# cloudflare/zkp-ecdsa

Measured on NVIDIA H100. Metric: ZKAttest proofs/sec, higher is better.
Workload: dtype u256/u258 (32-bit limbs, Montgomery)

## Files before the change

__graft_entry__.py:

```python
from __future__ import annotations

import hashlib
import os
import subprocess
import sys

ROOT = os.path.dirname(os.path.abspath(__file__))
CSRC = os.path.join(ROOT, 'zkp_ecdsa_b200', 'csrc')
LIB = os.path.join(ROOT, 'zkp_ecdsa_b200', 'libzkattest.so')
LIB_WAR = os.path.join(ROOT, 'zkp_ecdsa_b200', 'libzkattest_war256.so')
HOSTSIM = os.path.join(ROOT, 'tests', 'hostsim', 'libzkattest_hostsim.so')
HOSTSIM_WAR = os.path.join(ROOT, 'tests', 'hostsim', 'libzkattest_hostsim_war256.so')
PROBE_SRC = os.path.join(ROOT, 'tests', 'probe', 'zk_probe.cu')
PROBE = os.path.join(ROOT, 'tests', 'probe', 'libzkprobe.so')
PROBE_HOST = os.path.join(ROOT, 'tests', 'probe', 'libzkprobe_host.so')
ORACLE_CPU = os.path.join(ROOT, 'oracle', '_ref', 'libzkattest_cpu.so')
ARCH = ['-gencode', 'arch=compute_90a,code=sm_90a']
NVCC_FLAGS = ARCH + ['-O3', '-std=c++17', '-lineinfo',
              '--compiler-options', '-fPIC', '-shared']


def _sources():
    return sorted(os.path.join(CSRC, f) for f in os.listdir(CSRC) if f.endswith(('.cu', '.cuh', '.h', '.inc')))


def _stamp(extra='', files=()):
    h = hashlib.sha256(extra.encode())
    for p in _sources() + [os.path.join(ROOT, 'include', 'zkattest.h')] + list(files):
        h.update(p.encode())
        h.update(open(p, 'rb').read())
    return h.hexdigest()


def _build_if_stale(out, cmd, tag, files=()):
    stamp_file = out + '.stamp'
    stamp = _stamp(' '.join(cmd), files)
    if os.path.exists(out) and os.path.exists(stamp_file) and open(stamp_file).read() == stamp:
        return False
    print(f'[build] {tag}: {" ".join(cmd)}', flush=True)
    tmp = out + '.tmp'
    subprocess.check_call([tmp if c == out else c for c in cmd], cwd=ROOT)
    os.replace(tmp, out)
    open(stamp_file, 'w').write(stamp)
    return True


def build_lib():
    nvcc = os.environ.get('NVCC', '/usr/local/cuda/bin/nvcc')
    cmd = [nvcc] + NVCC_FLAGS + ['-I' + os.path.join(ROOT, 'include'), '-I' + CSRC, '-o', LIB,
                                 os.path.join(CSRC, 'zkattest.cu')]
    return _build_if_stale(LIB, cmd, 'libzkattest.so (sm_90a)')


def build_lib_war():
    nvcc = os.environ.get('NVCC', '/usr/local/cuda/bin/nvcc')
    cmd = [nvcc] + NVCC_FLAGS + ['-DZKA_PG_WAR256', '-I' + os.path.join(ROOT, 'include'), '-I' + CSRC, '-o', LIB_WAR,
                                 os.path.join(CSRC, 'zkattest.cu')]
    return _build_if_stale(LIB_WAR, cmd, 'libzkattest_war256.so (sm_90a)')


def build_hostsim(war=False):
    out = HOSTSIM_WAR if war else HOSTSIM
    os.makedirs(os.path.dirname(out), exist_ok=True)
    cmd = ['g++', '-std=c++17', '-O2', '-DZKA_HOSTSIM'] + (['-DZKA_PG_WAR256'] if war else []) + [
        '-x', 'c++', '-I' + os.path.join(ROOT, 'include'), '-I' + CSRC, '-fPIC', '-shared', '-o', out,
        os.path.join(CSRC, 'zkattest.cu')]
    return _build_if_stale(out, cmd, 'hostsim war256 (tests only)' if war else 'hostsim (tests only)')


def build_probe(host=False):
    out = PROBE_HOST if host else PROBE
    if host:
        cmd = ['g++', '-std=c++17', '-O2', '-DZKA_HOSTSIM', '-x', 'c++', '-fPIC', '-shared']
    else:
        cmd = [os.environ.get('NVCC', '/usr/local/cuda/bin/nvcc')] + NVCC_FLAGS
    cmd += ['-I' + os.path.join(ROOT, 'include'), '-I' + CSRC, '-o', out, PROBE_SRC]
    return _build_if_stale(out, cmd, 'probe host (tests only)' if host else 'probe (sm_90a, tests only)', [PROBE_SRC])


def build_oracle_cpu():
    src = os.path.join(ROOT, 'oracle', 'cpu', 'zkattest_cpu.cpp')
    hdr = os.path.join(ROOT, 'include', 'zkattest.h')
    if os.path.exists(ORACLE_CPU) and os.path.getmtime(ORACLE_CPU) >= max(os.path.getmtime(src), os.path.getmtime(hdr)):
        return False
    print('[build] oracle/cpu -> oracle/_ref/libzkattest_cpu.so', flush=True)
    subprocess.check_call(['make', '-C', os.path.join(ROOT, 'oracle', 'cpu')])
    return True


def build_tools():
    nvcc = os.environ.get('NVCC', '/usr/local/cuda/bin/nvcc')
    tdir = os.path.join(ROOT, 'tools')
    for name in ('imad_peak', 'mul_peak'):
        src, out = os.path.join(tdir, name + '.cu'), os.path.join(tdir, name)
        if not os.path.exists(src):
            continue
        if os.path.exists(out) and os.path.getmtime(out) >= max(os.path.getmtime(p) for p in _sources() + [src]):
            continue
        cmd = [nvcc] + ARCH + ['-O3', '-std=c++17', '-I' + CSRC,
               '-I' + os.path.join(ROOT, 'include'), '-o', out, src]
        print(f'[build] tools/{name}: {" ".join(cmd)}', flush=True)
        subprocess.check_call(cmd, cwd=ROOT)


def build() -> None:
    from concurrent.futures import ThreadPoolExecutor
    jobs = [build_lib, build_lib_war, build_hostsim, lambda: build_hostsim(war=True), build_oracle_cpu, build_tools,
            build_probe, lambda: build_probe(host=True)]
    with ThreadPoolExecutor(max_workers=min(len(jobs), max(1, (os.cpu_count() or 2)))) as ex:
        for f in [ex.submit(j) for j in jobs]:
            f.result()
    sys.path.insert(0, ROOT)
    import zkp_ecdsa_b200
    import oracle


def smoke() -> None:
    sys.path.insert(0, ROOT)
    import numpy as np
    from zkp_ecdsa_b200 import api, synth
    from oracle import flat
    from oracle import zkattest as OZ
    from oracle.big import Tape

    eng = api.Engine(device=0)
    rnd = synth.params_rnd(1)
    params = eng.generate_params_list(rnd=rnd)
    wl = synth.Workload(B=2, N=8, seed=1)
    tape = synth.random_tape(2, eng.lib.prove_tape_len(8), seed=2)
    res = eng.prove_batch(params, wl.msg_hash, wl.sig, wl.pk, wl.which, wl.ring, tape)
    assert (res.status == 0).all(), res.status
    oparams = OZ.generate_params_list(Tape(rnd))
    for b in range(2):
        pr = OZ.prove_signature_list(oparams, wl.msg_hash[b].tobytes(), wl.sig[b].tobytes(), wl.pk[b].tobytes(),
                                     int(wl.which[b]), wl.ring_ints(), Tape(tape[b].tobytes()))
        assert flat.ser_proof(pr) == res.proof_bytes(b), f'proof {b} differs from the oracle'
    from zkp_ecdsa_b200 import verify_tape as VT
    vts = eng.lib.verify_tape_len(8, 80)
    ok = np.zeros(2, np.uint8)
    st = np.zeros(2, np.int32)
    eng.lib.verify_batch(params.handle, 2, wl.msg_hash, wl.ring, 8, res.proofs, res.proofs.shape[1], res.proof_len,
                         VT.random_verify_tape(2, vts, 8, 80, seed=3), vts, ok, st)
    assert list(ok) == [1, 1] and not st.any(), (ok, st)
    launched = eng.lib.launch_count()
    war = ''
    if os.path.exists(LIB_WAR):
        from oracle.curves import tomEdwards256, war256
        ew = api.Engine(device=0, proof_group='war256')
        pw = ew.generate_params_list(16, rnd=rnd)
        tw = synth.random_tape(1, ew.lib.prove_tape_len(8, 16), seed=4)
        rw = ew.prove_batch(pw, wl.msg_hash[:1], wl.sig[:1], wl.pk[:1], wl.which[:1], wl.ring, tw)
        assert (rw.status == 0).all(), rw.status
        flat.set_proof_group(war256)
        try:
            ow = OZ.generate_params_list(Tape(rnd), 16, war256)
            pr = OZ.prove_signature_list(ow, wl.msg_hash[0].tobytes(), wl.sig[0].tobytes(), wl.pk[0].tobytes(),
                                         int(wl.which[0]), wl.ring_ints(), Tape(tw[0].tobytes()))
            assert flat.ser_proof(pr) == rw.proof_bytes(0), 'war256 proof differs from the oracle'
        finally:
            flat.set_proof_group(tomEdwards256)
        launched += ew.lib.launch_count()
        war = '; war256 build: 1 proof bit-exact'
    print(f'smoke ok: 2 proofs bit-exact vs oracle and accepted by the verifier{war}; kernels launched:', launched)


if __name__ == '__main__':
    build()
    if len(sys.argv) > 1 and sys.argv[1] == 'smoke':
        smoke()
```

zkp_ecdsa_b200/csrc/zk_field.cuh:

```cuda
#pragma once
#include <stdint.h>
#include "zk_field_consts.inc"

#if defined(__CUDACC__)
#define ZK_HD __host__ __device__ __forceinline__
#define ZK_HDN __host__ __device__ __noinline__
#else
#define ZK_HD inline __attribute__((always_inline))
#define ZK_HDN __attribute__((noinline))
#endif

namespace zk {

#define ZK_FIELD_DESC(NAME, PFX, NL, LAZY)                                   \
  struct NAME {                                                              \
    static constexpr int N = NL;                                             \
    static constexpr bool kLazy = LAZY;                                      \
    static constexpr uint32_t kN0Inv = PFX##_N0INV;                          \
    ZK_HD static constexpr uint32_t p(int i) {                               \
      constexpr uint32_t t[NL] = PFX##_P;                                    \
      return t[i];                                                           \
    }                                                                        \
    ZK_HD static constexpr uint32_t rr(int i) {                              \
      constexpr uint32_t t[NL] = PFX##_RR;                                   \
// ... 135 lines not shown
      uint32_t c = add_n<N>(s, a, b);
      uint32_t br = sub_p<F>(t, s);
      csel_n<N>(r, (c != 0) || (br == 0), t, s);
    }
  }
  ZK_HD static void sub(uint32_t* r, const uint32_t* a, const uint32_t* b) {
    if (F::kLazy) {
      uint32_t p8[N];
#pragma unroll
      for (int i = 0; i < N; i++) p8[i] = (F::p(i) << 3) | (i > 0 ? (F::p(i - 1) >> 29) : 0u);
      uint32_t t[N];
      add_n<N>(t, a, p8);
      sub_n<N>(r, t, b);
    } else {
      uint32_t s[N], t[N];
      uint32_t br = sub_n<N>(s, a, b);
      uint32_t pp[N];
#pragma unroll
      for (int i = 0; i < N; i++) pp[i] = F::p(i);
      add_n<N>(t, s, pp);
      csel_n<N>(r, br != 0, t, s);
    }
  }
  ZK_HD static void neg(uint32_t* r, const uint32_t* a) {
    uint32_t z[N];
    zero_n<N>(z);
    sub(r, z, a);
  }
  ZK_HD static void dbl(uint32_t* r, const uint32_t* a) { add(r, a, a); }

  ZK_HD static void mul(uint32_t* r, const uint32_t* a, const uint32_t* b) {
#if defined(__CUDA_ARCH__) && !defined(ZKA_NO_PTX_MUL)
    if (same_t<F, FpTom>::value) { ptx::tom_mul(r, a, b); return; }
    if (same_t<F, FpP256>::value) { ptx::p256_mul(r, a, b); return; }
    if (same_t<F, FpWar>::value) {
      ptx::V8 x, y;
#pragma unroll
      for (int i = 0; i < 8; i++) { x.v[i] = a[i]; y.v[i] = b[i]; }
      const ptx::V8 z = ptx::cios8_mul_fn<FpWar>(x, y);
#pragma unroll
      for (int i = 0; i < 8; i++) r[i] = z.v[i];
      return;
    }
#endif
    mul_generic(r, a, b);
  }
  ZK_HD static void mul_generic(uint32_t* r, const uint32_t* a, const uint32_t* b) {
    uint32_t t[N + 2];
#pragma unroll
    for (int i = 0; i < N + 2; i++) t[i] = 0;
#pragma unroll
    for (int i = 0; i < N; i++) {
      uint64_t c = 0;
      const uint32_t bi = b[i];
#pragma unroll
      for (int j = 0; j < N; j++) {
        uint64_t s = (uint64_t)a[j] * bi + t[j] + c;
        t[j] = (uint32_t)s;
        c = s >> 32;
      }
      uint64_t s = (uint64_t)t[N] + c;
      t[N] = (uint32_t)s;
      t[N + 1] = (uint32_t)(s >> 32);
      const uint32_t m = t[0] * F::kN0Inv;
      c = ((uint64_t)m * F::p(0) + t[0]) >> 32;
#pragma unroll
      for (int j = 1; j < N; j++) {
        uint64_t s2 = (uint64_t)m * F::p(j) + t[j] + c;
        t[j - 1] = (uint32_t)s2;
        c = s2 >> 32;
      }
      s = (uint64_t)t[N] + c;
      t[N - 1] = (uint32_t)s;
      t[N] = t[N + 1] + (uint32_t)(s >> 32);
    }
    if (F::kLazy) {
      copy_n<N>(r, t);
    } else {
      uint32_t u[N];
      uint32_t br = sub_p<F>(u, t);
      csel_n<N>(r, (t[N] != 0) || (br == 0), u, t);
    }
  }
  ZK_HD static void sqr(uint32_t* r, const uint32_t* a) { mul(r, a, a); }

  ZK_HD static void set_one(uint32_t* r) {
#pragma unroll
    for (int i = 0; i < N; i++) r[i] = F::one(i);
  }
  ZK_HD static void to_mont(uint32_t* r, const uint32_t* a) {
    uint32_t rr[N];
#pragma unroll
    for (int i = 0; i < N; i++) rr[i] = F::rr(i);
    mul(r, a, rr);
  }
  ZK_HD static void from_mont(uint32_t* r, const uint32_t* a) {
    uint32_t o[N];
    zero_n<N>(o);
    o[0] = 1;
    mul(r, a, o);
    if (F::kLazy) {
      uint32_t t[N], p2[N];
#pragma unroll
      for (int i = 0; i < N; i++) p2[i] = (F::p(i) << 1) | (i > 0 ? (F::p(i - 1) >> 31) : 0u);
      uint32_t br = sub_n<N>(t, r, p2);
      csel_n<N>(r, br == 0, t, r);
      br = sub_p<F>(t, r);
      csel_n<N>(r, br == 0, t, r);
    } else {
      reduce(r);
    }
  }
  ZK_HD static bool is_zero(const uint32_t* a) {
    uint32_t t[N];
    copy_n<N>(t, a);
    reduce(t);
    return is_zero_n<N>(t);
  }
  ZK_HD static bool eq(const uint32_t* a, const uint32_t* b) {
    uint32_t t[N], u[N];
    copy_n<N>(t, a);
    copy_n<N>(u, b);
    reduce(t);
    reduce(u);
    return eq_n<N>(t, u);
  }

  static ZK_HDN void inv_fermat(uint32_t* r, const uint32_t* a) {
    uint32_t e[N];
#pragma unroll
    for (int i = 0; i < N; i++) e[i] = F::p(i);
    e[0] -= 2;
    uint32_t acc[N], base[N];
    set_one(acc);
    copy_n<N>(base, a);
    int top = N * 32 - 1;
    while (top > 0 && !((e[top >> 5] >> (top & 31)) & 1)) top--;
#pragma unroll 1
    for (int bit = top; bit >= 0; bit--) {
      sqr(acc, acc);
      if ((e[bit >> 5] >> (bit & 31)) & 1) mul(acc, acc, base);
    }
    copy_n<N>(r, acc);
  }

  static ZK_HDN void inv(uint32_t* out, const uint32_t* a) {
    constexpr int L = N + 1;
    uint32_t u[L], v[L], r[L], s[L];
    {
      uint32_t t[N];
      copy_n<N>(t, a);
      reduce(t);
#pragma unroll
      for (int i = 0; i < N; i++) { u[i] = F::p(i); v[i] = t[i]; r[i] = 0; s[i] = 0; }
      u[N] = 0; v[N] = 0; r[N] = 0; s[N] = 0;
      s[0] = 1;
    }
    if (is_zero_n<L>(v)) { zero_n<N>(out); return; }
    int k = 0;
#pragma unroll 1
    while (!is_zero_n<L>(v)) {
      uint32_t dm[L], dn[L], sm[L];
      const uint32_t bor = sub_n<L>(dm, u, v);
      sub_n<L>(dn, v, u);
      add_n<L>(sm, r, s);
      const bool ue = (u[0] & 1u) == 0, ve = (v[0] & 1u) == 0;
      const bool gt = (bor == 0) && !is_zero_n<L>(dm);
// ... 101 lines not shown
```

zkp_ecdsa_b200/csrc/zk_field_ptx.cuh:

```cuda
#pragma once

#if defined(__CUDA_ARCH__)
namespace zk {
namespace ptx {

__device__ __forceinline__ void mac3(uint32_t& a0, uint32_t& a1, uint32_t& a2, uint32_t x, uint32_t y) {
  asm("mad.lo.cc.u32 %0, %3, %4, %0;\n\t"
      "madc.hi.cc.u32 %1, %3, %4, %1;\n\t"
      "addc.u32 %2, %2, 0;"
      : "+r"(a0), "+r"(a1), "+r"(a2)
      : "r"(x), "r"(y));
}
__device__ __forceinline__ void add3(uint32_t& a0, uint32_t& a1, uint32_t& a2, uint32_t lo, uint32_t hi) {
  asm("add.cc.u32 %0, %0, %3;\n\t"
      "addc.cc.u32 %1, %1, %4;\n\t"
      "addc.u32 %2, %2, 0;"
      : "+r"(a0), "+r"(a1), "+r"(a2)
      : "r"(lo), "r"(hi));
}
__device__ __forceinline__ void addw(uint32_t& a0, uint32_t& a1, uint32_t& a2, uint32_t w) {
  asm("add.cc.u32 %0, %0, %3;\n\t"
      "addc.cc.u32 %1, %1, 0;\n\t"
      "addc.u32 %2, %2, 0;"
      : "+r"(a0), "+r"(a1), "+r"(a2)
// ... 111 lines not shown
      "madc.hi.cc.u32 %3, %11, %13, %3;\n\t"
      "addc.cc.u32 %4, %4, %14;\n\t"
      "addc.cc.u32 %5, %5, %15;\n\t"
      "addc.cc.u32 %6, %6, %16;\n\t"
      "addc.cc.u32 %7, %7, %17;\n\t"
      "addc.cc.u32 %8, %8, %18;\n\t"
      "addc.u32 %9, %9, %19;"
      : "+r"(A[I]), "+r"(A[I + 1]), "+r"(A[I + 2]), "+r"(A[I + 3]), "+r"(A[I + 4]), "+r"(A[I + 5]), "+r"(A[I + 6]),
        "+r"(A[I + 7]), "+r"(A[I + 8]), "+r"(A[I + 9]), "+r"(A[I + 10])
      : "r"(m), "r"(P0), "r"(P2), "r"(s1), "r"(t1), "r"(s2), "r"(t2), "r"(lo3), "r"(hi3));
  asm("mad.lo.cc.u32 %0, %9, %10, %0;\n\t"
      "madc.hi.cc.u32 %1, %9, %10, %1;\n\t"
      "madc.lo.cc.u32 %2, %9, %11, %2;\n\t"
      "madc.hi.cc.u32 %3, %9, %11, %3;\n\t"
      "addc.cc.u32 %4, %4, 0;\n\t"
      "addc.cc.u32 %5, %5, 0;\n\t"
      "addc.cc.u32 %6, %6, %12;\n\t"
      "addc.cc.u32 %7, %7, %13;\n\t"
      "addc.u32 %8, %8, 0;"
      : "+r"(Bq[I + 1]), "+r"(Bq[I + 2]), "+r"(Bq[I + 3]), "+r"(Bq[I + 4]), "+r"(Bq[I + 5]), "+r"(Bq[I + 6]),
        "+r"(Bq[I + 7]), "+r"(Bq[I + 8]), "+r"(Bq[I + 9])
      : "r"(m), "r"(P1), "r"(P3), "r"(lo7), "r"(hi7));
}
__device__ __forceinline__ void tom_mul_body(uint32_t* r, const uint32_t* a, const uint32_t* b) {
  static_assert(FpTom::p(4) == 2 && FpTom::p(5) == 0 && FpTom::p(6) == 4 && FpTom::p(7) == 0xfffffffcu && FpTom::p(8) == 3,
                "tom.p limb structure");
  uint32_t E[20], O[20];
#pragma unroll
  for (int i = 0; i < 20; i++) { E[i] = 0; O[i] = 0; }
  tom_row<0, true>(E, O, a[0], b);
  tom_row<1, false>(O, E, a[1], b);
  tom_row<2, false>(E, O, a[2], b);
  tom_row<3, false>(O, E, a[3], b);
  tom_row<4, false>(E, O, a[4], b);
  tom_row<5, false>(O, E, a[5], b);
  tom_row<6, false>(E, O, a[6], b);
  tom_row<7, false>(O, E, a[7], b);
  tom_row<8, false>(E, O, a[8], b);
  asm("add.cc.u32 %0, %9, %18;\n\t"
      "addc.cc.u32 %1, %10, %19;\n\t"
      "addc.cc.u32 %2, %11, %20;\n\t"
      "addc.cc.u32 %3, %12, %21;\n\t"
      "addc.cc.u32 %4, %13, %22;\n\t"
      "addc.cc.u32 %5, %14, %23;\n\t"
      "addc.cc.u32 %6, %15, %24;\n\t"
      "addc.cc.u32 %7, %16, %25;\n\t"
      "addc.u32 %8, %17, %26;"
      : "=r"(r[0]), "=r"(r[1]), "=r"(r[2]), "=r"(r[3]), "=r"(r[4]), "=r"(r[5]), "=r"(r[6]), "=r"(r[7]), "=r"(r[8])
      : "r"(E[9]), "r"(E[10]), "r"(E[11]), "r"(E[12]), "r"(E[13]), "r"(E[14]), "r"(E[15]), "r"(E[16]), "r"(E[17]),
        "r"(O[9]), "r"(O[10]), "r"(O[11]), "r"(O[12]), "r"(O[13]), "r"(O[14]), "r"(O[15]), "r"(O[16]), "r"(O[17]));
}

__device__ __forceinline__ void p256_mul_body(uint32_t* r, const uint32_t* a, const uint32_t* b) {
  constexpr int N = 8;
  uint32_t m[N], t[N + 1];
  uint32_t a0 = 0, a1 = 0, a2 = 0;
#pragma unroll
  for (int k = 0; k < 2 * N; k++) {
#pragma unroll
    for (int i = 0; i < N; i++) {
      const int j = k - i;
      if (j >= 0 && j < N) mac3(a0, a1, a2, a[i], b[j]);
    }
    if (k - 3 >= 0 && k - 3 < N) addw(a0, a1, a2, m[k - 3 < 0 ? 0 : (k - 3 >= N ? 0 : k - 3)]);
    if (k - 6 >= 0 && k - 6 < N) addw(a0, a1, a2, m[k - 6 < 0 ? 0 : (k - 6 >= N ? 0 : k - 6)]);
    if (k - 7 >= 0 && k - 7 < N) subw(a0, a1, a2, m[k - 7 < 0 ? 0 : (k - 7 >= N ? 0 : k - 7)]);
    if (k - 8 >= 0 && k - 8 < N) addw(a0, a1, a2, m[k - 8 < 0 ? 0 : (k - 8 >= N ? 0 : k - 8)]);
    if (k < N) {
      m[k] = a0;
      a0 = 0;
    } else {
      t[k - N] = a0;
    }
    a0 = a1; a1 = a2; a2 = (uint32_t)((int32_t)a2 >> 31);
  }
  t[N] = a0;
  uint32_t u[N];
  uint32_t br = sub_p<FpP256>(u, t);
  const bool ge = (t[N] != 0) || (br == 0);
#pragma unroll
  for (int i = 0; i < N; i++) r[i] = ge ? u[i] : t[i];
}

template <int I, bool kFirst>
__device__ __forceinline__ void p256_row(uint32_t* A, uint32_t* Bq, uint32_t x, const uint32_t* b) {
  if (kFirst) {
    asm("mad.lo.cc.u32 %0, %9, %10, %0;\n\t"
        "madc.hi.cc.u32 %1, %9, %10, %1;\n\t"
        "madc.lo.cc.u32 %2, %9, %11, %2;\n\t"
        "madc.hi.cc.u32 %3, %9, %11, %3;\n\t"
        "madc.lo.cc.u32 %4, %9, %12, %4;\n\t"
        "madc.hi.cc.u32 %5, %9, %12, %5;\n\t"
        "madc.lo.cc.u32 %6, %9, %13, %6;\n\t"
        "madc.hi.cc.u32 %7, %9, %13, %7;\n\t"
        "addc.u32 %8, %8, 0;"
        : "+r"(Bq[I + 1]), "+r"(Bq[I + 2]), "+r"(Bq[I + 3]), "+r"(Bq[I + 4]), "+r"(Bq[I + 5]), "+r"(Bq[I + 6]),
          "+r"(Bq[I + 7]), "+r"(Bq[I + 8]), "+r"(Bq[I + 9])
        : "r"(x), "r"(b[1]), "r"(b[3]), "r"(b[5]), "r"(b[7]));
  } else {
    asm("add.cc.u32 %0, %0, %10;\n\t"
        "madc.lo.cc.u32 %1, %11, %12, %1;\n\t"
        "madc.hi.cc.u32 %2, %11, %12, %2;\n\t"
        "madc.lo.cc.u32 %3, %11, %13, %3;\n\t"
        "madc.hi.cc.u32 %4, %11, %13, %4;\n\t"
        "madc.lo.cc.u32 %5, %11, %14, %5;\n\t"
        "madc.hi.cc.u32 %6, %11, %14, %6;\n\t"
        "madc.lo.cc.u32 %7, %11, %15, %7;\n\t"
        "madc.hi.cc.u32 %8, %11, %15, %8;\n\t"
        "addc.u32 %9, %9, 0;"
        : "+r"(A[I]), "+r"(Bq[I + 1]), "+r"(Bq[I + 2]), "+r"(Bq[I + 3]), "+r"(Bq[I + 4]), "+r"(Bq[I + 5]),
          "+r"(Bq[I + 6]), "+r"(Bq[I + 7]), "+r"(Bq[I + 8]), "+r"(Bq[I + 9])
        : "r"(Bq[I]), "r"(x), "r"(b[1]), "r"(b[3]), "r"(b[5]), "r"(b[7]));
  }
  asm("mad.lo.cc.u32 %0, %9, %10, %0;\n\t"
      "madc.hi.cc.u32 %1, %9, %10, %1;\n\t"
      "madc.lo.cc.u32 %2, %9, %11, %2;\n\t"
      "madc.hi.cc.u32 %3, %9, %11, %3;\n\t"
      "madc.lo.cc.u32 %4, %9, %12, %4;\n\t"
      "madc.hi.cc.u32 %5, %9, %12, %5;\n\t"
      "madc.lo.cc.u32 %6, %9, %13, %6;\n\t"
      "madc.hi.cc.u32 %7, %9, %13, %7;\n\t"
      "addc.u32 %8, %8, 0;"
      : "+r"(A[I]), "+r"(A[I + 1]), "+r"(A[I + 2]), "+r"(A[I + 3]), "+r"(A[I + 4]), "+r"(A[I + 5]), "+r"(A[I + 6]),
        "+r"(A[I + 7]), "+r"(A[I + 8])
      : "r"(x), "r"(b[0]), "r"(b[2]), "r"(b[4]), "r"(b[6]));
  const uint32_t m = A[I];
  uint32_t negm, third;
  asm("sub.cc.u32 %0, 0, %2;\n\tsubc.u32 %1, %2, 0;" : "=r"(negm), "=r"(third) : "r"(m));
  asm("add.cc.u32 %0, %0, %7;\n\t"
      "addc.cc.u32 %1, %1, 0;\n\t"
      "addc.cc.u32 %2, %2, 0;\n\t"
      "addc.cc.u32 %3, %3, %7;\n\t"
      "addc.cc.u32 %4, %4, %8;\n\t"
      "addc.cc.u32 %5, %5, %9;\n\t"
      "addc.u32 %6, %6, 0;"
      : "+r"(A[I + 3]), "+r"(A[I + 4]), "+r"(A[I + 5]), "+r"(A[I + 6]), "+r"(A[I + 7]), "+r"(A[I + 8]), "+r"(A[I + 9])
      : "r"(m), "r"(negm), "r"(third));
}
__device__ __forceinline__ void p256_mul_body_os(uint32_t* r, const uint32_t* a, const uint32_t* b) {
  constexpr int N = 8;
  uint32_t E[18], O[18];
#pragma unroll
  for (int i = 0; i < 18; i++) { E[i] = 0; O[i] = 0; }
  p256_row<0, true>(E, O, a[0], b);
  p256_row<1, false>(O, E, a[1], b);
  p256_row<2, false>(E, O, a[2], b);
  p256_row<3, false>(O, E, a[3], b);
  p256_row<4, false>(E, O, a[4], b);
  p256_row<5, false>(O, E, a[5], b);
  p256_row<6, false>(E, O, a[6], b);
  p256_row<7, false>(O, E, a[7], b);
  uint32_t t[N + 1];
  asm("add.cc.u32 %0, %9, %18;\n\t"
      "addc.cc.u32 %1, %10, %19;\n\t"
      "addc.cc.u32 %2, %11, %20;\n\t"
      "addc.cc.u32 %3, %12, %21;\n\t"
      "addc.cc.u32 %4, %13, %22;\n\t"
      "addc.cc.u32 %5, %14, %23;\n\t"
      "addc.cc.u32 %6, %15, %24;\n\t"
      "addc.cc.u32 %7, %16, %25;\n\t"
      "addc.u32 %8, %17, %26;"
      : "=r"(t[0]), "=r"(t[1]), "=r"(t[2]), "=r"(t[3]), "=r"(t[4]), "=r"(t[5]), "=r"(t[6]), "=r"(t[7]), "=r"(t[8])
      : "r"(E[8]), "r"(E[9]), "r"(E[10]), "r"(E[11]), "r"(E[12]), "r"(E[13]), "r"(E[14]), "r"(E[15]), "r"(E[16]),
        "r"(O[8]), "r"(O[9]), "r"(O[10]), "r"(O[11]), "r"(O[12]), "r"(O[13]), "r"(O[14]), "r"(O[15]), "r"(O[16]));
  uint32_t u[N];
  uint32_t br = sub_p<FpP256>(u, t);
  const bool ge = (t[N] != 0) || (br == 0);
#pragma unroll
  for (int i = 0; i < N; i++) r[i] = ge ? u[i] : t[i];
}

struct V9 { uint32_t v[9]; };
struct V8 { uint32_t v[8]; };
static __device__ __noinline__ V9 tom_mul_fn(V9 a, V9 b) {
  V9 r;
  tom_mul_body(r.v, a.v, b.v);
  return r;
}
static __device__ __noinline__ V8 p256_mul_fn(V8 a, V8 b) {
  V8 r;
  p256_mul_body(r.v, a.v, b.v);
  return r;
}
__device__ __forceinline__ void tom_mul(uint32_t* r, const uint32_t* a, const uint32_t* b) {
#if defined(ZKA_INLINE_MUL)
  tom_mul_body(r, a, b);
#else
  V9 x, y;
#pragma unroll
  for (int i = 0; i < 9; i++) { x.v[i] = a[i]; y.v[i] = b[i]; }
  V9 z = tom_mul_fn(x, y);
#pragma unroll
  for (int i = 0; i < 9; i++) r[i] = z.v[i];
#endif
}
__device__ __forceinline__ void p256_mul(uint32_t* r, const uint32_t* a, const uint32_t* b) {
#if defined(ZKA_INLINE_MUL)
  p256_mul_body(r, a, b);
#else
  V8 x, y;
#pragma unroll
  for (int i = 0; i < 8; i++) { x.v[i] = a[i]; y.v[i] = b[i]; }
  V8 z = p256_mul_fn(x, y);
#pragma unroll
  for (int i = 0; i < 8; i++) r[i] = z.v[i];
#endif
}

}
}
#endif
```

zkp_ecdsa_b200/csrc/zk_prove.cuh:

```cuda
#pragma once
#include "zk_sigma.cuh"

namespace zk {

struct ProveCtx {
  int B;
  int S;
  int N;
  int n;
  int M;
  int tom_w, tom_nwin;
  int mode;
  int head_len;
  const uint8_t* base;
  const uint8_t* s_in;
  const uint8_t* q_in;
  uint32_t* base_aff;
  const uint8_t* msg_hash;
  const uint8_t* sig;
  const uint8_t* pk;
  const uint32_t* which;
  uint32_t* which_s;
  const uint8_t* tape;
  size_t tape_stride;
// ... 170 lines not shown
    uint32_t s1[8], z1[8];
    Fn::mul(t, sinv, zm); st<8>(c.u12 + (size_t)b * 16, t);
    Fn::mul(t, sinv, rm); st<8>(c.u12 + (size_t)b * 16 + 8, t);
    Fn::mul(t, rinv, sm); Fn::from_mont(s1, t);
    Fn::mul(t, rinv, zm); Fn::from_mont(z1, t);
    st<8>(c.s1 + (size_t)b * 8, s1);

    P256Pt Q;
    p256_set_identity(Q);
    p256_accum_fixed(Q, c.g_tab8, z1, 8);
    uint32_t zi[8];
    P256Aff Qa;
    bool qinf = p256_is_identity(Q);
    if (qinf) {
      p256_set_generator(Qa);
    } else {
      Fp::inv(zi, Q.z);
      Fp::mul(Qa.x, Q.x, zi);
      Fp::mul(Qa.y, Q.y, zi);
    }
    p256_st_aff(c.q_aff + (size_t)b * 16, Qa);
    c.q_inf[b] = qinf ? 1 : 0;
  }
};

struct KeyDedupTask {
  ProveCtx c;
  ZK_HD void operator()(int b) const {
    uint32_t mine[16];
    ld<16>(mine, c.base_aff + (size_t)b * 16);
    int rep = b;
    for (int o = 0; o < b; o++) {
      const uint32_t* q = c.base_aff + (size_t)o * 16;
      if (q[0] != mine[0]) continue;
      bool same = true;
      for (int i = 1; i < 16; i++) same = same && (q[i] == mine[i]);
      if (same) { rep = o; break; }
    }
    c.tab_of[b] = (uint32_t)rep;
  }
};
struct KeyRankTask {
  ProveCtx c;
  ZK_HD void operator()(int b) const {
    const uint32_t rep = c.tab_of[b];
    uint32_t rank = 0;
    for (uint32_t o = 0; o < rep; o++) rank += (c.tab_of[o] == o) ? 1u : 0u;
    c.tab_rep[c.B + b] = rank;
    if (rep == (uint32_t)b) c.tab_rep[rank] = (uint32_t)b;
    if (b == c.B - 1) {
      uint32_t total = 0;
      for (uint32_t o = 0; o < (uint32_t)c.B; o++) total += (c.tab_of[o] == o) ? 1u : 0u;
      c.tab_count[0] = total;
      c.tab_count[1] = (uint32_t)key_window_bits(total, (uint32_t)c.B, (uint32_t)c.S + 2);
    }
  }
};
struct KeyAssignTask {
  ProveCtx c;
  ZK_HD void operator()(int b) const { c.tab_of[b] = c.tab_rep[c.B + b]; }
};

struct PowsAndPreTask {
  P256PowsTask pows;
  PreTask pre;
  int Bp;
  ZK_HD void operator()(int t) const {
    if (t < Bp) {
      if (t < pows.nbase) pows(t);
    } else if (t - Bp < pre.c.B) {
      pre(t - Bp);
    }
  }
};

struct RPointTask {
  ProveCtx c;
  ZK_HD void operator()(int b) const {
    using Fp = P256p;
    using Fn = P256n;
    uint32_t m[8], u1[8], u2[8];
    ld<8>(m, c.u12 + (size_t)b * 16);     Fn::from_mont(u1, m);
    ld<8>(m, c.u12 + (size_t)b * 16 + 8); Fn::from_mont(u2, m);
    P256Pt R;
    p256_set_identity(R);
    p256_accum_fixed(R, c.g_tabw, u1, c.g_w);
    const int kw = (int)c.tab_count[1];
    p256_accum_fixed(R, c.rtab + (size_t)c.tab_of[b] * key_table_words(kw), u2, kw);
    uint32_t zi[8];
    P256Aff Ra;
    if (p256_is_identity(R)) {
      ZK_SET_STATUS_OVER(c.status + b, ZKA_ERR_T_INFINITY, ZKA_ERR_TAPE_RANGE);
      p256_set_generator(Ra);
    } else {
      Fp::inv(zi, R.z);
      Fp::mul(Ra.x, R.x, zi);
      Fp::mul(Ra.y, R.y, zi);
    }
    if (c.mode == 0) {
      uint32_t r[8];
      limbs_from_be<8>(r, c.sig + (size_t)b * 64, 32);
      reduce_once<FnP256>(r);
      if (is_zero_n<8>(r)) ZK_SET_STATUS_OVER(c.status + b, ZKA_ERR_POINTS_DONT_ADD, ZKA_ERR_TAPE_RANGE);
    }
    p256_st_aff(c.r_aff + (size_t)b * 16, Ra);
    uint8_t* rb = c.r_bytes + (size_t)b * BSTRIDE;
    uint32_t cv[8];
    rb[0] = 0x04;
    Fp::from_mont(cv, Ra.x); limbs_to_be<8>(rb + 1, cv, 32);
    Fp::from_mont(cv, Ra.y); limbs_to_be<8>(rb + 33, cv, 32);
    if (c.mode == 0 && c.which[b] >= (uint32_t)c.N) ZK_SET_STATUS_OVER(c.status + b, ZKA_ERR_BAD_INDEX, ZKA_ERR_TAPE_RANGE);
  }
};

struct PhaseAP256Task {
  ProveCtx c;
  ZK_HD void operator()(int t) const {
    using Fn = P256n;
    const int S1 = c.S + 1;
    const int b = t / S1, i = t % S1;
    uint32_t alpha[8], r[8];
    if (i < c.S) {
      draw_checked<FnP256>(alpha, c, b, DRAW_REP0 + DRAWS_PER_REP * i);
      draw_checked<FnP256>(r, c, b, DRAW_REP0 + DRAWS_PER_REP * i + 1);
    } else {
      ld<8>(alpha, c.s1 + (size_t)b * 8);
      draw_checked<FnP256>(r, c, b, DRAW_COMS1_R);
    }
    uint32_t am[8], um[8], pm[8], a1[8], a2[8];
    Fn::to_mont(am, alpha);
    ld<8>(um, c.u12 + (size_t)b * 16);     Fn::mul(pm, am, um); Fn::from_mont(a1, pm);
    ld<8>(um, c.u12 + (size_t)b * 16 + 8); Fn::mul(pm, am, um); Fn::from_mont(a2, pm);
    P256Pt T, A;
    p256_set_identity(T);
    p256_accum_fixed(T, c.g_tabw, a1, c.g_w);
    const int kw = (int)c.tab_count[1];
    p256_accum_fixed(T, c.rtab + (size_t)c.tab_of[b] * key_table_words(kw), a2, kw);
    A = T;
    p256_accum_fixed(A, c.h_tab8, r, c.h_w);
    p256_st_proj(c.pa_T + (size_t)t * P256_PROJ_WORDS, T);
    p256_st_proj(c.pa_A + (size_t)t * P256_PROJ_WORDS, A);
  }
};


struct PhaseAAndRPointTask {
  PhaseAP256Task pa;
  RPointTask rp;
  int nA, nAp;
  ZK_HD void operator()(int t) const {
    if (t < nAp) {
      if (t < nA) pa(t);
    } else if (t - nAp < rp.c.B) {
      rp(t - nAp);
    }
  }
};

struct JobsATask {
  ProveCtx c;
  ZK_HD void operator()(int t) const {
    using Fp = P256p;
    const int per = 2 + 2 * c.S;
    const int b = t / per, j = t % per;
    uint32_t v[8], r[8], m[8];
    if (j < 2) {
      ld8v(m, c.pk_aff + (size_t)b * 16 + 8 * j);
      draw_checked<FpP256>(r, c, b, DRAW_PKX_R + j);
    } else {
      const int i = (j - 2) >> 1, xy = (j - 2) & 1;
      const size_t slot = (size_t)b * (c.S + 1) + i;
      if (c.pa_T_inf[slot]) ZK_SET_STATUS(c.status + b, ZKA_ERR_T_INFINITY);
      if (c.pa_A_inf[slot]) ZK_SET_STATUS(c.status + b, ZKA_ERR_IDENTITY_ENC);
      ld8v(m, c.pa_T_aff + slot * 16 + 8 * xy);
      draw_checked<FpP256>(r, c, b, DRAW_REP0 + DRAWS_PER_REP * i + 2 + xy);
    }
    Fp::from_mont(v, m);
    st8v(c.s1_jv + (size_t)t * 8, v);
    st8v(c.s1_jr + (size_t)t * 8, r);
  }
};

struct ExpChallengeTask {
  ProveCtx c;
  struct Src {
    const ProveCtx* c;
    int b;
    ZK_HD const uint8_t* operator()(int k, int& len) const {
      if (k < 2) { len = WP; return c->s1_bytes + c->s1_pt(b, k) * BSTRIDE; }
      const int i = (k - 2) / 3, w = (k - 2) % 3;
      if (w == 0) { len = NP; return c->pa_A_bytes + ((size_t)b * (c->S + 1) + i) * BSTRIDE; }
      len = WP;
      return c->s1_bytes + c->s1_pt(b, 2 + 2 * i + (w - 1)) * BSTRIDE;
    }
  };
  ZK_HD void operator()(int b) const {
    uint32_t c3[3];
    Src src{&c, b};
    hash_points80(c3, src, 2 + 3 * c.S);
    st<3>(c.chal + (size_t)b * 3, c3);
    uint32_t off = (uint32_t)c.head_len, z = 0;
    for (int i = 0; i < c.S; i++) {
      const uint32_t bit = (c3[i >> 5] >> (i & 31)) & 1u;
      c.rep_off[(size_t)b * c.S + i] = off;
      off += bit ? REP1_LEN : REP0_LEN;
      z += bit ? 0 : 1;
    }
    c.zcount[b] = z;
    c.gk_off[b] = off;
    c.proof_len[b] = c.mode == 1 ? off : off + gk_len(c.n);
  }
};
struct ScanTask {
  ProveCtx c;
  ZK_HD void operator()(int) const {
    uint32_t acc = 0, mx = 0;
    for (int b = 0; b < c.B; b++) {
      c.item_base[b] = acc;
      acc += c.zcount[b];
      if (c.zcount[b] > mx) mx = c.zcount[b];
    }
    c.item_total[0] = acc;
// ... 835 lines not shown
```

zkp_ecdsa_b200/csrc/zk_weier.inc:

```
struct WEI_PT {
  uint32_t x[8], y[8], z[8];
};
struct WEI_AFF {
  uint32_t x[8], y[8];
};

ZK_HD void WEI_FN(const_b)(uint32_t* r) {
  constexpr uint32_t t[8] = WEI_B_MONT;
#pragma unroll
  for (int i = 0; i < 8; i++) r[i] = t[i];
}
ZK_HD void WEI_FN(set_identity)(WEI_PT& p) {
  zero_n<8>(p.x);
  WEI_F::set_one(p.y);
  zero_n<8>(p.z);
}
ZK_HD void WEI_FN(set_generator)(WEI_AFF& g) {
  constexpr uint32_t gx[8] = WEI_GX_MONT;
  constexpr uint32_t gy[8] = WEI_GY_MONT;
#pragma unroll
  for (int i = 0; i < 8; i++) {
    g.x[i] = gx[i];
    g.y[i] = gy[i];
  }
// ... 34 lines not shown
  F::sub(y3, y3, z3);
  F::add(x3, y3, y3);
  F::add(y3, x3, y3);
  F::sub(x3, t1, y3);
  F::add(y3, t1, y3);
  F::mul(y3, x3, y3);
  F::mul(x3, x3, t3);
  F::add(t3, t2, t2);
  F::add(t2, t2, t3);
  F::mul(z3, b, z3);
  F::sub(z3, z3, t2);
  F::sub(z3, z3, t0);
  F::add(t3, z3, z3);
  F::add(z3, z3, t3);
  F::add(t3, t0, t0);
  F::add(t0, t3, t0);
  F::sub(t0, t0, t2);
  F::mul(t0, t0, z3);
  F::add(y3, y3, t0);
  F::mul(t0, p.y, p.z);
  F::add(t0, t0, t0);
  F::mul(z3, t0, z3);
  F::sub(x3, x3, z3);
  F::mul(z3, t0, t1);
  F::add(z3, z3, z3);
  F::add(z3, z3, z3);
  copy_n<8>(r.x, x3);
  copy_n<8>(r.y, y3);
  copy_n<8>(r.z, z3);
}

struct WEI_JAC {
  uint32_t x[8], y[8], z[8];
};
ZK_HD void WEI_FN(jac_dbl)(WEI_JAC& r, const WEI_JAC& p) {
  using F = WEI_F;
  uint32_t delta[8], gamma[8], beta[8], alpha[8], t0[8], t1[8];
  F::sqr(delta, p.z);
  F::sqr(gamma, p.y);
  F::mul(beta, p.x, gamma);
  F::sub(t0, p.x, delta);
  F::add(t1, p.x, delta);
  F::mul(alpha, t0, t1);
  F::add(t0, alpha, alpha);
  F::add(alpha, t0, alpha);
  F::add(t0, p.y, p.z);
  F::sqr(t0, t0);
  F::sub(t0, t0, gamma);
  F::sub(r.z, t0, delta);
  F::add(t0, beta, beta);
  F::add(t0, t0, t0);
  F::add(t1, t0, t0);
  F::sqr(r.x, alpha);
  F::sub(r.x, r.x, t1);
  F::sub(t0, t0, r.x);
  F::mul(t0, alpha, t0);
  F::sqr(t1, gamma);
  F::add(t1, t1, t1);
  F::add(t1, t1, t1);
  F::add(t1, t1, t1);
  F::sub(r.y, t0, t1);
}
ZK_HD void WEI_FN(jac_to_hom)(WEI_PT& r, const WEI_JAC& p) {
  using F = WEI_F;
  uint32_t z2[8];
  F::sqr(z2, p.z);
  F::mul(r.x, p.x, p.z);
  copy_n<8>(r.y, p.y);
  F::mul(r.z, z2, p.z);
}
ZK_HD void WEI_FN(hom_to_jac)(WEI_JAC& r, const WEI_PT& p) {
  using F = WEI_F;
  uint32_t z2[8];
  F::sqr(z2, p.z);
  F::mul(r.x, p.x, p.z);
  F::mul(r.y, p.y, z2);
  copy_n<8>(r.z, p.z);
  if (is_zero_n<8>(p.z)) {
    F::set_one(r.x);
    F::set_one(r.y);
  }
}

ZK_HD void WEI_FN(dbl_n)(WEI_PT& p, int c) {
  WEI_JAC q;
  WEI_FN(hom_to_jac)(q, p);
  for (int i = 0; i < c; i++) WEI_FN(jac_dbl)(q, q);
  WEI_FN(jac_to_hom)(p, q);
}

ZK_HD void WEI_FN(add_tail)(WEI_PT& r, uint32_t* t0, uint32_t* t1, uint32_t* t2, uint32_t* t3, uint32_t* t4,
                         uint32_t* y3) {
  using F = WEI_F;
  uint32_t x3[8], z3[8], b[8];
  WEI_FN(const_b)(b);
  F::mul(z3, b, t2);
  F::sub(x3, y3, z3);
  F::add(z3, x3, x3);
  F::add(x3, x3, z3);
  F::sub(z3, t1, x3);
  F::add(x3, t1, x3);
  F::mul(y3, b, y3);
  F::add(t1, t2, t2);
  F::add(t2, t1, t2);
  F::sub(y3, y3, t2);
  F::sub(y3, y3, t0);
  F::add(t1, y3, y3);
  F::add(y3, t1, y3);
  F::add(t1, t0, t0);
  F::add(t0, t1, t0);
  F::sub(t0, t0, t2);
  F::mul(t1, t4, y3);
  F::mul(t2, t0, y3);
  F::mul(y3, x3, z3);
  F::add(y3, y3, t2);
  F::mul(x3, t3, x3);
  F::sub(x3, x3, t1);
  F::mul(z3, t4, z3);
  F::mul(t1, t3, t0);
  F::add(z3, z3, t1);
  copy_n<8>(r.x, x3);
  copy_n<8>(r.y, y3);
  copy_n<8>(r.z, z3);
}

ZK_HD void WEI_FN(add)(WEI_PT& r, const WEI_PT& p, const WEI_PT& q) {
  using F = WEI_F;
  uint32_t t0[8], t1[8], t2[8], t3[8], t4[8], x3[8], y3[8];
  F::mul(t0, p.x, q.x);
  F::mul(t1, p.y, q.y);
  F::mul(t2, p.z, q.z);
  F::add(t3, p.x, p.y);
  F::add(t4, q.x, q.y);
  F::mul(t3, t3, t4);
  F::add(t4, t0, t1);
  F::sub(t3, t3, t4);
  F::add(t4, p.y, p.z);
  F::add(x3, q.y, q.z);
  F::mul(t4, t4, x3);
  F::add(x3, t1, t2);
  F::sub(t4, t4, x3);
  F::add(x3, p.x, p.z);
  F::add(y3, q.x, q.z);
  F::mul(x3, x3, y3);
  F::add(y3, t0, t2);
  F::sub(y3, x3, y3);
  WEI_FN(add_tail)(r, t0, t1, t2, t3, t4, y3);
}

ZK_HD void WEI_FN(madd)(WEI_PT& r, const WEI_PT& p, const WEI_AFF& q) {
  using F = WEI_F;
  uint32_t t0[8], t1[8], t2[8], t3[8], t4[8], y3[8];
  F::mul(t0, p.x, q.x);
  F::mul(t1, p.y, q.y);
  F::add(t3, p.x, p.y);
  F::add(t4, q.x, q.y);
  F::mul(t3, t3, t4);
  F::add(t4, t0, t1);
  F::sub(t3, t3, t4);
  F::mul(t4, q.y, p.z);
  F::add(t4, t4, p.y);
  F::mul(y3, q.x, p.z);
  F::add(y3, y3, p.x);
  copy_n<8>(t2, p.z);
  WEI_FN(add_tail)(r, t0, t1, t2, t3, t4, y3);
}
// ... 2 lines not shown
```

zkp_ecdsa_b200/csrc/zk_weier_ops.inc:

```
ZK_HD void WEI_FN(ld_proj)(WEI_PT& p, const uint32_t* m) {
  ld<8>(p.x, m); ld<8>(p.y, m + 8); ld<8>(p.z, m + 16);
}
ZK_HD void WEI_FN(st_proj)(uint32_t* m, const WEI_PT& p) {
  st<8>(m, p.x); st<8>(m + 8, p.y); st<8>(m + 16, p.z);
}
ZK_HD void WEI_FN(ld_aff)(WEI_AFF& a, const uint32_t* m) { ld<8>(a.x, m); ld<8>(a.y, m + 8); }
ZK_HD void WEI_FN(st_aff)(uint32_t* m, const WEI_AFF& a) { st<8>(m, a.x); st<8>(m + 8, a.y); }

struct WEI_T(PowsTask) {
  const uint32_t* base_aff;
  const uint8_t* base_inf;
  uint32_t* pows;
  int nbase, nwin, w;
  const uint32_t* index = nullptr;
  const uint32_t* count_dev = nullptr;
  const uint32_t* w_dev = nullptr;
  ZK_HD void operator()(int t) const {
    if (count_dev && (uint32_t)t >= *count_dev) return;
    const int w = w_dev ? (int)*w_dev : this->w;
    const int nwin = w_dev ? fb_windows(w) : this->nwin;
    const size_t src = index ? index[t] : (size_t)t;
    WEI_AFF a;
    WEI_FN(ld_aff)(a, base_aff + src * P256_AFF_WORDS);
    WEI_PT p;
// ... 76 lines not shown
  }
};
struct WEI_T(RowsLoTask) {
  const uint32_t* pows;
  const uint32_t* hi;
  uint32_t* rows;
  int w;
  ZK_HD void operator()(int t) const {
    const int nh = 1 << (w - 9);
    const int j = t / nh, m = t % nh;
    WEI_PT p, acc;
    WEI_FN(ld_proj)(p, pows + (size_t)j * P256_PROJ_WORDS);
    WEI_FN(ld_proj)(acc, hi + (size_t)t * P256_PROJ_WORDS);
    uint32_t* out = rows + ((size_t)j * fb_entries(w) + ((size_t)m << 8)) * P256_PROJ_WORDS;
    for (int d = 0; d < 256; d++) {
      WEI_FN(st_proj)(out + (size_t)d * P256_PROJ_WORDS, acc);
      WEI_FN(add)(acc, acc, p);
    }
  }
};

struct WEI_T(NormTask) {
  const uint32_t* proj;
  uint32_t* aff;
  uint8_t* bytes;
  uint8_t* inf;
  int count;
  int chunk;
  const uint32_t* groups_dev = nullptr;
  int group_size = 0;
  const uint32_t* w_dev = nullptr;
  ZK_HD void operator()(int t) const {
    using F = WEI_F;
    const int lo = t * chunk;
    int total = count;
    const int group_size = w_dev ? fb_windows((int)*w_dev) * fb_entries((int)*w_dev) : this->group_size;
    if (groups_dev) {
      const long long present = (long long)*groups_dev * group_size;
      if (present < total) total = (int)present;
    }
    int n = total - lo;
    if (n > chunk) n = chunk;
    if (n <= 0) return;
    uint32_t pre[NORM_CHUNK_MAX][8];
    uint32_t acc[8], z[8], one[8];
    F::set_one(one);
    copy_n<8>(acc, one);
    for (int k = 0; k < n; k++) {
      ld<8>(z, proj + (size_t)(lo + k) * P256_PROJ_WORDS + 16);
      if (is_zero_n<8>(z)) copy_n<8>(z, one);
      F::mul(acc, acc, z);
      copy_n<8>(pre[k], acc);
    }
    uint32_t inv[8];
    F::inv(inv, acc);
    for (int k = n - 1; k >= 0; k--) {
      const uint32_t* src = proj + (size_t)(lo + k) * P256_PROJ_WORDS;
      ld<8>(z, src + 16);
      const bool isinf = is_zero_n<8>(z);
      if (isinf) copy_n<8>(z, one);
      uint32_t zi[8];
      if (k > 0) F::mul(zi, inv, pre[k - 1]); else copy_n<8>(zi, inv);
      F::mul(inv, inv, z);
      WEI_AFF a;
      uint32_t X[8], Y[8];
      ld<8>(X, src);
      ld<8>(Y, src + 8);
      F::mul(a.x, X, zi);
      F::mul(a.y, Y, zi);
      WEI_FN(st_aff)(aff + (size_t)(lo + k) * P256_AFF_WORDS, a);
      if (inf) inf[lo + k] = isinf ? 1 : 0;
      if (bytes) {
        uint8_t* o = bytes + (size_t)(lo + k) * BSTRIDE;
        uint32_t cx[8], cy[8];
        F::from_mont(cx, a.x);
        F::from_mont(cy, a.y);
        if (isinf) { zero_n<8>(cx); zero_n<8>(cy); }
        store_point_words<8, 32>(o, isinf ? 0x00u : 0x04u, cx, cy);
      }
    }
  }
};

ZK_HD void WEI_FN(accum_fixed)(WEI_PT& acc, const uint32_t* tab, const uint32_t* k, int w) {
  const int nwin = fb_windows(w);
  const size_t E = (size_t)fb_entries(w);
  uint32_t carry = 0;
  for (int j = 0; j < nwin; j++) {
    bool neg;
    const uint32_t d = signed_digit(k, j, w, carry, neg);
    if (d) {
      WEI_AFF q;
      WEI_FN(ld_aff)(q, tab + ((size_t)j * E + d) * P256_AFF_WORDS);
      if (neg) WEI_F::neg(q.y, q.y);
      WEI_FN(madd)(acc, acc, q);
    }
  }
}
```

Measured before the change: 105,300.

## Accumulate fixed-base multiplications in Jacobian coordinates with dedicated P-256 squaring

Fixed-base scalar accumulation now uses a Jacobian mixed-add (madd-2007-bl style) instead of the homogeneous projective madd, converting to homogeneous only at the end. The prover's R, T and A computations keep one Jacobian accumulator across tables. A PTX squaring routine for the P-256 field computes the off-diagonal products once and doubles them, and is used by F::sqr. The intent is fewer field multiplications per point addition. The cost is extra branches in the Jacobian madd and new code paths that must stay bit-exact with the oracle.

Result: faster. 109,000, median of 6 (+3.5%).

```diff
diff --git a/__graft_entry__.py b/__graft_entry__.py
--- a/__graft_entry__.py
+++ b/__graft_entry__.py
@@ -14,6 +14,9 @@
 PROBE_SRC = os.path.join(ROOT, 'tests', 'probe', 'zk_probe.cu')
 PROBE = os.path.join(ROOT, 'tests', 'probe', 'libzkprobe.so')
 PROBE_HOST = os.path.join(ROOT, 'tests', 'probe', 'libzkprobe_host.so')
+PROBE_JAC_SRC = os.path.join(ROOT, 'tests', 'probe', 'zk_probe_jac.cu')
+PROBE_JAC = os.path.join(ROOT, 'tests', 'probe', 'libzkprobe_jac.so')
+PROBE_JAC_HOST = os.path.join(ROOT, 'tests', 'probe', 'libzkprobe_jac_host.so')
 ORACLE_CPU = os.path.join(ROOT, 'oracle', '_ref', 'libzkattest_cpu.so')
 ARCH = ['-gencode', 'arch=compute_90a,code=sm_90a']
 NVCC_FLAGS = ARCH + ['-O3', '-std=c++17', '-lineinfo',
@@ -68,14 +71,16 @@
     return _build_if_stale(out, cmd, 'hostsim war256 (tests only)' if war else 'hostsim (tests only)')
 
 
-def build_probe(host=False):
-    out = PROBE_HOST if host else PROBE
+def build_probe(host=False, jac=False):
+    out = (PROBE_JAC_HOST if host else PROBE_JAC) if jac else (PROBE_HOST if host else PROBE)
+    src = PROBE_JAC_SRC if jac else PROBE_SRC
     if host:
         cmd = ['g++', '-std=c++17', '-O2', '-DZKA_HOSTSIM', '-x', 'c++', '-fPIC', '-shared']
     else:
         cmd = [os.environ.get('NVCC', '/usr/local/cuda/bin/nvcc')] + NVCC_FLAGS
-    cmd += ['-I' + os.path.join(ROOT, 'include'), '-I' + CSRC, '-o', out, PROBE_SRC]
-    return _build_if_stale(out, cmd, 'probe host (tests only)' if host else 'probe (sm_90a, tests only)', [PROBE_SRC])
+    cmd += ['-I' + os.path.join(ROOT, 'include'), '-I' + CSRC, '-o', out, src]
+    tag = ('probe_jac' if jac else 'probe') + (' host (tests only)' if host else ' (sm_90a, tests only)')
+    return _build_if_stale(out, cmd, tag, [PROBE_SRC, PROBE_JAC_SRC] if jac else [PROBE_SRC])
 
 
 def build_oracle_cpu():
@@ -106,7 +111,8 @@
 def build() -> None:
     from concurrent.futures import ThreadPoolExecutor
     jobs = [build_lib, build_lib_war, build_hostsim, lambda: build_hostsim(war=True), build_oracle_cpu, build_tools,
-            build_probe, lambda: build_probe(host=True)]
+            build_probe, lambda: build_probe(host=True), lambda: build_probe(jac=True),
+            lambda: build_probe(host=True, jac=True)]
     with ThreadPoolExecutor(max_workers=min(len(jobs), max(1, (os.cpu_count() or 2)))) as ex:
         for f in [ex.submit(j) for j in jobs]:
             f.result()
diff --git a/zkp_ecdsa_b200/csrc/zk_field.cuh b/zkp_ecdsa_b200/csrc/zk_field.cuh
--- a/zkp_ecdsa_b200/csrc/zk_field.cuh
+++ b/zkp_ecdsa_b200/csrc/zk_field.cuh
@@ -241,7 +241,12 @@
       csel_n<N>(r, (t[N] != 0) || (br == 0), u, t);
     }
   }
-  ZK_HD static void sqr(uint32_t* r, const uint32_t* a) { mul(r, a, a); }
+  ZK_HD static void sqr(uint32_t* r, const uint32_t* a) {
+#if defined(__CUDA_ARCH__) && !defined(ZKA_NO_PTX_MUL)
+    if (same_t<F, FpP256>::value) { ptx::p256_sqr(r, a); return; }
+#endif
+    mul(r, a, a);
+  }
 
   ZK_HD static void set_one(uint32_t* r) {
 #pragma unroll
diff --git a/zkp_ecdsa_b200/csrc/zk_field_ptx.cuh b/zkp_ecdsa_b200/csrc/zk_field_ptx.cuh
--- a/zkp_ecdsa_b200/csrc/zk_field_ptx.cuh
+++ b/zkp_ecdsa_b200/csrc/zk_field_ptx.cuh
@@ -217,6 +217,48 @@
   for (int i = 0; i < N; i++) r[i] = ge ? u[i] : t[i];
 }
 
+__device__ __forceinline__ void p256_sqr_body(uint32_t* r, const uint32_t* a) {
+  constexpr int N = 8;
+  uint32_t m[N], t[N + 1];
+  uint32_t a0 = 0, a1 = 0, a2 = 0;
+#pragma unroll
+  for (int k = 0; k < 2 * N; k++) {
+    if (k >= 1 && k <= 2 * N - 3) {
+      uint32_t c0 = 0, c1 = 0, c2 = 0;
+#pragma unroll
+      for (int i = 0; i < N; i++) {
+        const int j = k - i;
+        if (i < j && j < N) mac3(c0, c1, c2, a[i], a[j]);
+      }
+      asm("add.cc.u32 %0, %0, %0;\n\t"
+          "addc.cc.u32 %1, %1, %1;\n\t"
+          "addc.u32 %2, %2, %2;\n\t"
+          "add.cc.u32 %3, %3, %0;\n\t"
+          "addc.cc.u32 %4, %4, %1;\n\t"
+          "addc.u32 %5, %5, %2;"
+          : "+r"(c0), "+r"(c1), "+r"(c2), "+r"(a0), "+r"(a1), "+r"(a2));
+    }
+    if ((k & 1) == 0 && k / 2 < N) mac3(a0, a1, a2, a[k / 2], a[k / 2]);
+    if (k - 3 >= 0 && k - 3 < N) addw(a0, a1, a2, m[k - 3 < 0 ? 0 : (k - 3 >= N ? 0 : k - 3)]);
+    if (k - 6 >= 0 && k - 6 < N) addw(a0, a1, a2, m[k - 6 < 0 ? 0 : (k - 6 >= N ? 0 : k - 6)]);
+    if (k - 7 >= 0 && k - 7 < N) subw(a0, a1, a2, m[k - 7 < 0 ? 0 : (k - 7 >= N ? 0 : k - 7)]);
+    if (k - 8 >= 0 && k - 8 < N) addw(a0, a1, a2, m[k - 8 < 0 ? 0 : (k - 8 >= N ? 0 : k - 8)]);
+    if (k < N) {
+      m[k] = a0;
+      a0 = 0;
+    } else {
+      t[k - N] = a0;
+    }
+    a0 = a1; a1 = a2; a2 = (uint32_t)((int32_t)a2 >> 31);
+  }
+  t[N] = a0;
+  uint32_t u[N];
+  uint32_t br = sub_p<FpP256>(u, t);
+  const bool ge = (t[N] != 0) || (br == 0);
+#pragma unroll
+  for (int i = 0; i < N; i++) r[i] = ge ? u[i] : t[i];
+}
+
 template <int I, bool kFirst>
 __device__ __forceinline__ void p256_row(uint32_t* A, uint32_t* Bq, uint32_t x, const uint32_t* b) {
   if (kFirst) {
@@ -317,6 +359,11 @@
   p256_mul_body(r.v, a.v, b.v);
   return r;
 }
+static __device__ __noinline__ V8 p256_sqr_fn(V8 a) {
+  V8 r;
+  p256_sqr_body(r.v, a.v);
+  return r;
+}
 __device__ __forceinline__ void tom_mul(uint32_t* r, const uint32_t* a, const uint32_t* b) {
 #if defined(ZKA_INLINE_MUL)
   tom_mul_body(r, a, b);
@@ -341,7 +388,19 @@
   for (int i = 0; i < 8; i++) r[i] = z.v[i];
 #endif
 }
-
-}
-}
+__device__ __forceinline__ void p256_sqr(uint32_t* r, const uint32_t* a) {
+#if defined(ZKA_INLINE_MUL)
+  p256_sqr_body(r, a);
+#else
+  V8 x;
+#pragma unroll
+  for (int i = 0; i < 8; i++) x.v[i] = a[i];
+  V8 z = p256_sqr_fn(x);
+#pragma unroll
+  for (int i = 0; i < 8; i++) r[i] = z.v[i];
 #endif
+}
+
+}
+}
+#endif
diff --git a/zkp_ecdsa_b200/csrc/zk_prove.cuh b/zkp_ecdsa_b200/csrc/zk_prove.cuh
--- a/zkp_ecdsa_b200/csrc/zk_prove.cuh
+++ b/zkp_ecdsa_b200/csrc/zk_prove.cuh
@@ -276,11 +276,13 @@
     uint32_t m[8], u1[8], u2[8];
     ld<8>(m, c.u12 + (size_t)b * 16);     Fn::from_mont(u1, m);
     ld<8>(m, c.u12 + (size_t)b * 16 + 8); Fn::from_mont(u2, m);
+    P256Jac acc;
+    p256_set_identity_jac(acc);
+    p256_accum_fixed_jac(acc, c.g_tabw, u1, c.g_w);
+    const int kw = (int)c.tab_count[1];
+    p256_accum_fixed_jac(acc, c.rtab + (size_t)c.tab_of[b] * key_table_words(kw), u2, kw);
     P256Pt R;
-    p256_set_identity(R);
-    p256_accum_fixed(R, c.g_tabw, u1, c.g_w);
-    const int kw = (int)c.tab_count[1];
-    p256_accum_fixed(R, c.rtab + (size_t)c.tab_of[b] * key_table_words(kw), u2, kw);
+    p256_jac_to_hom(R, acc);
     uint32_t zi[8];
     P256Aff Ra;
     if (p256_is_identity(R)) {
@@ -325,13 +327,15 @@
     Fn::to_mont(am, alpha);
     ld<8>(um, c.u12 + (size_t)b * 16);     Fn::mul(pm, am, um); Fn::from_mont(a1, pm);
     ld<8>(um, c.u12 + (size_t)b * 16 + 8); Fn::mul(pm, am, um); Fn::from_mont(a2, pm);
+    P256Jac acc;
+    p256_set_identity_jac(acc);
+    p256_accum_fixed_jac(acc, c.g_tabw, a1, c.g_w);
+    const int kw = (int)c.tab_count[1];
+    p256_accum_fixed_jac(acc, c.rtab + (size_t)c.tab_of[b] * key_table_words(kw), a2, kw);
     P256Pt T, A;
-    p256_set_identity(T);
-    p256_accum_fixed(T, c.g_tabw, a1, c.g_w);
-    const int kw = (int)c.tab_count[1];
-    p256_accum_fixed(T, c.rtab + (size_t)c.tab_of[b] * key_table_words(kw), a2, kw);
-    A = T;
-    p256_accum_fixed(A, c.h_tab8, r, c.h_w);
+    p256_jac_to_hom(T, acc);
+    p256_accum_fixed_jac(acc, c.h_tab8, r, c.h_w);
+    p256_jac_to_hom(A, acc);
     p256_st_proj(c.pa_T + (size_t)t * P256_PROJ_WORDS, T);
     p256_st_proj(c.pa_A + (size_t)t * P256_PROJ_WORDS, A);
   }
diff --git a/zkp_ecdsa_b200/csrc/zk_weier.inc b/zkp_ecdsa_b200/csrc/zk_weier.inc
--- a/zkp_ecdsa_b200/csrc/zk_weier.inc
+++ b/zkp_ecdsa_b200/csrc/zk_weier.inc
@@ -140,6 +140,52 @@
   }
 }
 
+ZK_HD void WEI_FN(jac_madd)(WEI_JAC& r, const WEI_JAC& p, const WEI_AFF& q) {
+  using F = WEI_F;
+  if (is_zero_n<8>(p.z)) {
+    copy_n<8>(r.x, q.x);
+    copy_n<8>(r.y, q.y);
+    F::set_one(r.z);
+    return;
+  }
+  uint32_t z1z1[8], u2[8], s2[8], h[8], rr[8], hh[8], i4[8], j[8], v[8], t0[8];
+  F::sqr(z1z1, p.z);
+  F::mul(u2, q.x, z1z1);
+  F::mul(t0, p.z, z1z1);
+  F::mul(s2, q.y, t0);
+  F::sub(h, u2, p.x);
+  F::sub(rr, s2, p.y);
+  F::add(rr, rr, rr);
+  if (is_zero_n<8>(h)) {
+    if (is_zero_n<8>(rr)) {
+      WEI_FN(jac_dbl)(r, p);
+    } else {
+      F::set_one(r.x);
+      F::set_one(r.y);
+      zero_n<8>(r.z);
+    }
+    return;
+  }
+  F::sqr(hh, h);
+  F::add(i4, hh, hh);
+  F::add(i4, i4, i4);
+  F::mul(j, h, i4);
+  F::mul(v, p.x, i4);
+  F::add(t0, p.z, h);
+  F::sqr(t0, t0);
+  F::sub(t0, t0, z1z1);
+  F::sub(r.z, t0, hh);
+  F::mul(t0, p.y, j);
+  F::add(t0, t0, t0);
+  F::sqr(r.x, rr);
+  F::sub(r.x, r.x, j);
+  F::sub(r.x, r.x, v);
+  F::sub(r.x, r.x, v);
+  F::sub(v, v, r.x);
+  F::mul(v, rr, v);
+  F::sub(r.y, v, t0);
+}
+
 ZK_HD void WEI_FN(dbl_n)(WEI_PT& p, int c) {
   WEI_JAC q;
   WEI_FN(hom_to_jac)(q, p);
diff --git a/zkp_ecdsa_b200/csrc/zk_weier_ops.inc b/zkp_ecdsa_b200/csrc/zk_weier_ops.inc
--- a/zkp_ecdsa_b200/csrc/zk_weier_ops.inc
+++ b/zkp_ecdsa_b200/csrc/zk_weier_ops.inc
@@ -182,7 +182,7 @@
   }
 };
 
-ZK_HD void WEI_FN(accum_fixed)(WEI_PT& acc, const uint32_t* tab, const uint32_t* k, int w) {
+ZK_HD void WEI_FN(accum_fixed_jac)(WEI_JAC& acc, const uint32_t* tab, const uint32_t* k, int w) {
   const int nwin = fb_windows(w);
   const size_t E = (size_t)fb_entries(w);
   uint32_t carry = 0;
@@ -193,7 +193,18 @@
       WEI_AFF q;
       WEI_FN(ld_aff)(q, tab + ((size_t)j * E + d) * P256_AFF_WORDS);
       if (neg) WEI_F::neg(q.y, q.y);
-      WEI_FN(madd)(acc, acc, q);
-    }
-  }
-}
+      WEI_FN(jac_madd)(acc, acc, q);
+    }
+  }
+}
+ZK_HD void WEI_FN(accum_fixed)(WEI_PT& acc, const uint32_t* tab, const uint32_t* k, int w) {
+  WEI_JAC q;
+  WEI_FN(hom_to_jac)(q, acc);
+  WEI_FN(accum_fixed_jac)(q, tab, k, w);
+  WEI_FN(jac_to_hom)(acc, q);
+}
+ZK_HD void WEI_FN(set_identity_jac)(WEI_JAC& p) {
+  WEI_F::set_one(p.x);
+  WEI_F::set_one(p.y);
+  zero_n<8>(p.z);
+}
```
